# talmolab/VNL-Brax-Imitation

Measured on AMD Instinct MI355X. Metric: env-steps/sec (whole node), rodent imitation, num_envs=4096/GPU, higher is better.
Workload: dtype f32; 1 GPU; rodent imitation rollout, single groom clip, 4096 envs/GPU: intention-policy forward (HIP) -> RodentTracking.step (5 substeps, CG 6/6) -> auto-reset on -> Transition logging (unroll 20, the 20 steps replayed as one captured hipGraph); envs_per_gpu=4096, clips=1, parallelism=env-sharded x1, no data-path collective

## Files before the change

### __graft_entry__.py

```python
from __future__ import annotations

import os
import sys

ROOT = os.path.dirname(os.path.abspath(__file__))
if ROOT not in sys.path:
    sys.path.insert(0, ROOT)


def build() -> None:
    import vnl_brax_imitation_amd
    from vnl_brax_imitation_amd.csrc import build as hip_build

    from concurrent.futures import ThreadPoolExecutor

    with ThreadPoolExecutor(6) as pool:
        futs = {v: pool.submit(hip_build.build, variant=v) for v in ("product", "spill", "noblk", "nospec", "tail", "plain")}
        paths = {v: f.result() for v, f in futs.items()}
    path = paths["product"]
    assert all(os.path.exists(p_) for p_ in paths.values()), paths
    from oracle import oracle as _oracle

    _oracle.build()
    from vnl_brax_imitation_amd import _lib

    _lib.load_library(path)
    print(f"[build] {path} ok; oracle ok")


def smoke() -> None:
    import numpy as np
    import torch

    sys.path.insert(0, os.path.join(ROOT, "tests"))
    import helpers as H
    from vnl_brax_imitation_amd.envs.rodent import RodentTracking

    assert torch.cuda.is_available(), "smoke() needs a HIP device"
    B = 256
    env = RodentTracking(H.reference_clip(), num_envs=B, device="cuda:0", **H.env_kwargs())
# ... 43 lines not shown
```

### vnl-brax-imitation_amd/csrc/build.py

```python
from __future__ import annotations

import os
import subprocess
import sys

HERE = os.path.dirname(os.path.abspath(__file__))
SOURCES = ["vnl_lib.hip", "vnl_policy.hip", "vnl_ppo.hip", "vnl_domain.hip"]
DEPS = SOURCES + ["vnl_env_kernels.h", "vnl_body.h", "vnl_types.h", "vnl_philox.h", "vnl_policy_train.h", "../../include/vnl.h"]
OUT = os.path.join(HERE, "libvnl.so")

VARIANTS = {
    "product": ("libvnl.so", ["-DVNL_KERNEL_ATTR=__attribute__((amdgpu_waves_per_eu(2,2)))"]),
    "prof": ("libvnl_prof.so", ["-DVNL_PROFILE", "-DVNL_KERNEL_ATTR=__attribute__((amdgpu_waves_per_eu(2,2)))"]),
    "knobs": ("libvnl_knobs.so", ["-DVNL_STAGE_KNOBS", "-DVNL_KERNEL_ATTR=__attribute__((amdgpu_waves_per_eu(2,2)))"]),
    "spill": ("libvnl_spill.so", ["-DVNL_KERNEL_ATTR=__attribute__((amdgpu_waves_per_eu(4,4)))"]),
    "noblk": ("libvnl_noblk.so", ["-DVNL_NO_BLK", "-DVNL_KERNEL_ATTR=__attribute__((amdgpu_waves_per_eu(2,2)))"]),
    "tail": ("libvnl_tail.so", ["-DVNL_SOLVER_TAIL", "-DVNL_KERNEL_ATTR=__attribute__((amdgpu_waves_per_eu(2,2)))"]),
    "plain": ("libvnl_plain.so", ["-DVNL_SOLVER_PLAIN", "-DVNL_KERNEL_ATTR=__attribute__((amdgpu_waves_per_eu(2,2)))"]),
    "nospec": ("libvnl_nospec.so", ["-DVNL_NO_SPEC", "-DVNL_KERNEL_ATTR=__attribute__((amdgpu_waves_per_eu(2,2)))"]),
}
ENV_KERNELS = ("vnl_step_kernel", "vnl_reset_kernel", "vnl_reset_done_kernel")


def resource_usage(stderr_text: str) -> dict:
    out, name = {}, None
    for line in stderr_text.splitlines():
        if "Function Name:" in line:
            name = line.split("Function Name:")[1].split()[0]
            out[name] = {}
        elif name and "remark:" in line:
            body = line.split("remark:")[1].split("[-Rpass")[0].strip()
            key, _, val = body.rpartition(":")
            try:
                out[name][key.strip()] = int(val.strip())
            except ValueError:
                pass
    return out


def build(force: bool = False, verbose: bool = False, profile: bool = False, knobs: bool = False,
          variant: str | None = None) -> str:
# ... 78 lines not shown
```

### vnl-brax-imitation_amd/csrc/vnl_body.h

```cpp
#pragma once
#include <math.h>

#include "vnl_types.h"

#ifndef VNL_HD
#define VNL_HD __device__ __forceinline__
#endif
#include "vnl_philox.h"

#ifndef VNL_FORKJOIN_DEFINED
#define VNL_LANES 64
#define VNL_ROWS_PER_LANE 8
#define VNL_ROWS_SMALL 5
#define VNL_CHAIN_WIDTH 8
#define VNL_ROWSETS_1 1
#define VNL_ROWSETS_2 2
#define VNL_FOR(i, n) for (int i = (int)lane; i < (n); i += VNL_LANES)
#define VNL_SERIAL if (lane == 0)
#define VNL_SYNC() __builtin_amdgcn_fence(__ATOMIC_ACQ_REL, "wavefront")
#define VNL_SYNC_GLOBAL()                                     \
  do {                                                        \
    __builtin_amdgcn_fence(__ATOMIC_ACQ_REL, "wavefront");    \
    asm volatile("s_waitcnt vmcnt(0)" ::: "memory");          \
    __builtin_amdgcn_fence(__ATOMIC_ACQ_REL, "wavefront");    \
// ... 134 lines not shown
  return V3{m.a[0] * v.x + m.a[1] * v.y + m.a[2] * v.z, m.a[3] * v.x + m.a[4] * v.y + m.a[5] * v.z,
            m.a[6] * v.x + m.a[7] * v.y + m.a[8] * v.z};
}
struct S6 {
  V3 a, l;
};
VNL_HD S6 operator+(S6 p, S6 q) { return S6{p.a + q.a, p.l + q.l}; }
VNL_HD S6 operator*(S6 p, vreal s) { return S6{p.a * s, p.l * s}; }
VNL_HD vreal dot(S6 p, S6 q) { return dot(p.a, q.a) + dot(p.l, q.l); }
VNL_HD S6 mcross(S6 u, S6 v) { return S6{cross(u.a, v.a), cross(u.l, v.a) + cross(u.a, v.l)}; }
VNL_HD S6 mcross_force(S6 v, S6 f) { return S6{cross(v.a, f.a) + cross(v.l, f.l), cross(v.a, f.l)}; }

#if defined(__HIP_DEVICE_COMPILE__)
#define VNL_CAS __attribute__((address_space(4)))
#define VNL_TO_CAS(T, p) ((const VNL_CAS T*)(unsigned long long)(p))
#define VNL_LAUNDER(p) asm volatile("" : "+s"(p))
#else
#define VNL_CAS
#define VNL_TO_CAS(T, p) ((const T*)(p))
#define VNL_LAUNDER(p)
#endif
#define MI(f) (SP::fixed ? SP::D.f : m.f)
#define LO(f) (SP::fixed ? SP::L.f : L.f)
#if defined(__HIP_DEVICE_COMPILE__) && !defined(VNL_SOLVER_PLAIN)
#define VNL_SOLVE_REGS 1
#else
#define VNL_SOLVE_REGS 0
#endif
#define VNL_BLK_REGS 2
#define VNL_LIMROW_REGS 2
#define VNL_SR_BLK 1
#define VNL_SR_LIMROW 2
struct VnlSolveRegs {
  int on;
  unsigned blk[2][VNL_BLK_REGS];
  int limrow[VNL_LIMROW_REGS];
};
template <class SP>
struct EnvWaveT {
  const VNL_CAS DevModel& m;
  const VNL_CAS DevEnv& ev;
  const DevState& st;
  const VNL_CAS WsLayout& L;
  vreal* s;
  unsigned e, lane;
  const VNL_CAS KernelConsts* kc;
// ... 55 lines not shown

  VNL_HD V3 ld3(int o) const { return V3{s[o], s[o + 1], s[o + 2]}; }
  VNL_HD void st3(int o, V3 v) const { s[o] = v.x, s[o + 1] = v.y, s[o + 2] = v.z; }
  VNL_HD Q4 ld4(int o) const { return Q4{s[o], s[o + 1], s[o + 2], s[o + 3]}; }
  VNL_HD S6 ld6(int o) const { return S6{ld3(o), ld3(o + 3)}; }
  VNL_HD void st6(int o, S6 v) const { st3(o, v.a), st3(o + 3, v.l); }
  VNL_HD static V3 t3(const vreal* t, int i) { return V3{t[3 * i], t[3 * i + 1], t[3 * i + 2]}; }
  VNL_HD static Q4 t4(const vreal* t, int i) { return Q4{t[4 * i], t[4 * i + 1], t[4 * i + 2], t[4 * i + 3]}; }

  VNL_HD S6 inert_mul(int o, S6 v) const {
    vreal ixx = s[o], iyy = s[o + 1], izz = s[o + 2], ixy = s[o + 3], ixz = s[o + 4], iyz = s[o + 5];
    V3 mp = ld3(o + 6);
    vreal mass = s[o + 9];
    V3 ang = V3{ixx * v.a.x + ixy * v.a.y + ixz * v.a.z, ixy * v.a.x + iyy * v.a.y + iyz * v.a.z,
                ixz * v.a.x + iyz * v.a.y + izz * v.a.z} +
             cross(mp, v.l);
    V3 lin = v.l * mass - cross(mp, v.a);
    return S6{ang, lin};
  }

  VNL_HD vreal* gxpos() const { return st.xpos + (size_t)e * 3 * MI(nbody_out); }
  VNL_HD vreal* gxquat() const { return st.xquat + (size_t)e * 4 * MI(nbody_out); }
  VNL_HD vreal* gqfrc_act() const { return st.qfrc_actuator + (size_t)e * MI(nv); }
  VNL_HD vreal* fac2() const { return ev.fac2 + (size_t)e * (MI(nM) + MI(nv)); }
  enum { P_MU, P_INVW, P_GAIN, P_DAMP, P_ARM, P_MASS, P_IPOS, P_INERTIA6 };
  template <int F>
  VNL_HD vreal par(int i) const {
    if constexpr (SP::dom) {
      const VNL_CAS DevDomain& d = kc->dom;
      if constexpr (F == P_MU) return d.cg_mu[(size_t)e * MI(ncg) + i];
      else if constexpr (F == P_INVW) return d.cg_invweight[(size_t)e * MI(ncg) + i];
      else if constexpr (F == P_GAIN) return d.act_gain[(size_t)e * MI(nu) + i];
      else if constexpr (F == P_DAMP) return d.dof_damping[(size_t)e * MI(nv) + i];
      else return d.dof_armature[(size_t)e * MI(nv) + i];
    } else {
      if constexpr (F == P_MU) return m.cg_mu[i];
      else if constexpr (F == P_INVW) return m.cg_invweight[i];
      else if constexpr (F == P_GAIN) return m.act_gain[i];
      else if constexpr (F == P_DAMP) return m.dof_damping[i];
      else return m.dof_armature[i];
    }
  }
  template <int F>
  VNL_HD const vreal* par_row() const {
    if constexpr (SP::dom) {
      const VNL_CAS DevDomain& d = kc->dom;
      if constexpr (F == P_MASS) return d.body_mass + (size_t)e * MI(nbody);
// ... 590 lines not shown
#pragma unroll
          for (int u = 1; u < t; u++) acc -= nn[u] * x[u];
          nn[t] = acc;
        }
      }
      VNL_SYNC();
#pragma unroll
      for (int t = 1; t < MAXD; t++)
        if (t < qd(q) && t <= d) s[own + t] = nn[t];
      VNL_SYNC();
    }
  }

  template <int NSET>
  VNL_HD void factor_aba(vreal h) const {
    constexpr int LW = 16;
    const int sc = (LO(Mgrad) + 3) & ~3;
    const int VS = vstore();
    vreal* g2 = fac2();
    const int nsteps = MI(fac_steps);
    v2r U[NSET][6], diag[NSET];
    vreal S[NSET][6];
    int dep[NSET], ftime[NSET], myline[NSET], adrs[NSET];
    const unsigned char* mt[NSET];
    unsigned nxt[NSET];
#pragma unroll
    for (int q = 0; q < NSET; q++) {
      const int a = (int)lane + q * VNL_LANES;
      const bool ok = a < MI(nv);
      const int aa = ok ? a : 0;
      const S6 c = ld6(LO(cdof) + 6 * aa), f = inert_mul(LO(P) + 10 * m.dof_body[aa], c);
      S[q][0] = c.a.x, S[q][1] = c.a.y, S[q][2] = c.a.z, S[q][3] = c.l.x, S[q][4] = c.l.y, S[q][5] = c.l.z;
      U[q][0] = v2r{f.a.x, f.a.x}, U[q][1] = v2r{f.a.y, f.a.y}, U[q][2] = v2r{f.a.z, f.a.z};
      U[q][3] = v2r{f.l.x, f.l.x}, U[q][4] = v2r{f.l.y, f.l.y}, U[q][5] = v2r{f.l.z, f.l.z};
      const vreal arm = par<P_ARM>(aa);
      diag[q] = v2r{arm, arm + h * par<P_DAMP>(aa)};
      adrs[q] = madr(aa), dep[q] = eadr(aa) - adrs[q];
      myline[q] = m.dof_fslot[aa];
      ftime[q] = ok ? m.dof_ftime[aa] : -1;
      mt[q] = m.fac_match + (size_t)aa * nsteps;
      nxt[q] = (ok && nsteps > 0) ? mt[q][0] : 0u;
    }
    VNL_SYNC();
    VNL_PROF(7);
    for (int step = 0; step < nsteps; step++) {
      unsigned cur[NSET];
#pragma unroll
      for (int q = 0; q < NSET; q++) {
        cur[q] = nxt[q];
        nxt[q] = (ftime[q] >= 0 && step + 1 < nsteps) ? mt[q][step + 1] : 0u;
        if (ftime[q] == step) {
          const int a = (int)lane + q * VNL_LANES;
          v2r D = diag[q];
#pragma unroll
          for (int i = 0; i < 6; i++) D += v2r{S[q][i], S[q][i]} * U[q][i];
          const v2r iv = v2r{vnl_recip(D[0]), vnl_recip(D[1])};
          vreal* ln = s + sc + myline[q] * LW;
          st4a(ln, U[q][0][0], U[q][0][1], U[q][1][0], U[q][1][1]);
          st4a(ln + 4, U[q][2][0], U[q][2][1], U[q][3][0], U[q][3][1]);
          st4a(ln + 8, U[q][4][0], U[q][4][1], U[q][5][0], U[q][5][1]);
          st4a(ln + 12, iv[0], iv[1], (vreal)(adrs[q] + dep[q]), vreal(0.));
          vreal* vs = s + VS + 12 * a;
          const v2r v0 = U[q][0] * iv, v1 = U[q][1] * iv, v2 = U[q][2] * iv, v3_ = U[q][3] * iv, v4 = U[q][4] * iv, v5 = U[q][5] * iv;
          st4a(vs, v0[0], v0[1], v1[0], v1[1]);
          st4a(vs + 4, v2[0], v2[1], v3_[0], v3_[1]);
          st4a(vs + 8, v4[0], v4[1], v5[0], v5[1]);
          s[LO(dinv) + a] = iv[0];
          g2[MI(nM) + a] = iv[1];
        }
      }
      VNL_WAVE_FENCE();
      for (int pass = 0; pass < VNL_FAC_LINES; pass++) {
        bool more = false;
#pragma unroll
        for (int q = 0; q < NSET; q++) more = more || cur[q] != 0u;
        if (!vnl_wave_any(more)) break;
#pragma unroll
        for (int q = 0; q < NSET; q++) {
          if (cur[q] != 0u) {
            const int k = __builtin_ctz(cur[q]);
            cur[q] &= cur[q] - 1u;
            const vreal* ln = s + sc + k * LW;
            const R4 u0 = ld4a(ln), u1 = ld4a(ln + 4), u2 = ld4a(ln + 8), hd = ld4a(ln + 12);
            const v2r Uk[6] = {v2r{u0.x, u0.y}, v2r{u0.z, u0.w}, v2r{u1.x, u1.y}, v2r{u1.z, u1.w}, v2r{u2.x, u2.y}, v2r{u2.z, u2.w}};
            v2r pa = v2r{S[q][0], S[q][0]} * Uk[0], pb = v2r{S[q][1], S[q][1]} * Uk[1];
            pa += v2r{S[q][2], S[q][2]} * Uk[2], pb += v2r{S[q][3], S[q][3]} * Uk[3];
            pa += v2r{S[q][4], S[q][4]} * Uk[4], pb += v2r{S[q][5], S[q][5]} * Uk[5];
            const v2r Lk = (pa + pb) * v2r{hd.x, hd.y};
#pragma unroll
            for (int i = 0; i < 6; i++) U[q][i] -= Lk * Uk[i];
            s[LO(LD) + (int)hd.z - dep[q]] = Lk[0];
          }
        }
      }
      VNL_WAVE_FENCE();
    }
    VNL_SYNC();
    VNL_PROF(8);
    VNL_PROF(9);
  }

  VNL_HD int vstore() const { return vnl_vstore(LO(P)); }
  VNL_HD int cvel_at() const { return vnl_cvel_at(LO(P), LO(smooth), MI(nbody), MI(nv)); }

  template <int NSET, bool GUESTS>
  VNL_HD void invert_aba(vreal* g2) const {
    const int VS = vstore();
    const unsigned char* an = (const unsigned char*)(s + LO(tab_anc));
    auto load_v = [&](int r, v2r* C) {
      const vreal* vs = s + VS + 12 * r;
      const R4 a = ld4a(vs), b = ld4a(vs + 4), c = ld4a(vs + 8);
      C[0] = v2r{a.x, a.y}, C[1] = v2r{a.z, a.w}, C[2] = v2r{b.x, b.y}, C[3] = v2r{b.z, b.w}, C[4] = v2r{c.x, c.y}, C[5] = v2r{c.z, c.w};
    };
#pragma unroll
    for (int q = 0; q < NSET; q++) {
      const int a = (int)lane + q * VNL_LANES;
      int row = a < MI(nv) ? a : -1, next = -1;
      if (GUESTS && q == 0 && m.fac_guest) next = m.fac_guest[lane];
      int adr = madr(row >= 0 ? row : 0), d = row >= 0 ? eadr(row) - adr : 0, tt = 0;
// ... 302 lines not shown
    VNL_FOR(b, MI(nbody)) st6(ca + 6 * b, path_sum(QB, m.body_pathseg + 8 * b + 4));
    VNL_SYNC();
    VNL_PROF(3);
    VNL_FOR(b, MI(nbody)) {
      if (b == 0) {
        st6(ca, S6{v3(0, 0, 0), v3(0, 0, 0)});
        continue;
      }
      S6 vel = ld6(cv + 6 * b), acc = ld6(ca + 6 * b);
      acc.l = acc.l + v3(-m.gx, -m.gy, -m.gz);
      st6(ca + 6 * b, inert_mul(LO(P) + 10 * b, acc) + mcross_force(vel, inert_mul(LO(P) + 10 * b, vel)));
    }
    VNL_SYNC();
    tree_accumulate(ca, 6);
    VNL_FOR(d, MI(nv))
      s[LO(smooth) + d] = -par<P_DAMP>(d) * s[LO(qvel) + d] - dot(ld6(LO(cdof) + 6 * d), ld6(ca + 6 * m.dof_body[d]));
    VNL_SYNC();
    VNL_PROF(4);
    return cv;
  }

  VNL_HD void smooth_forces() const {
    VNL_FOR(j, MI(njnt)) {
      if (m.jnt_type[j] == VNL_JNT_HINGE) {
        vreal k = m.jnt_stiffness[j];
        if (k != vreal(0.)) s[LO(smooth) + m.jnt_dofadr[j]] -= k * (s[LO(qpos) + m.jnt_qposadr[j]] - m.jnt_springref[j]);
      }
    }
    const int frc = LO(tmp2), adof = LO(tmp);
    const bool listed = m.dof_act != nullptr;
    VNL_FOR(i, MI(nu)) {
      vreal ctrl = s[LO(ctrl) + i], a = ctrl;
      vreal tau = m.act_tau[i];
      if (tau >= vreal(0.)) {
        a = s[LO(act) + i];
        s[LO(actdot) + i] = (ctrl - a) / fmax(tau, VNL_MINVAL);
      }
      s[frc + i] = m.act_gear[i] * par<P_GAIN>(i) * a;
      if (!listed) s[adof + i] = vreal(m.act_dof[i]);
    }
    VNL_SYNC();
    vreal* gf = gqfrc_act();
    VNL_FOR(d, MI(nv)) {
      vreal fa = vreal(0.);
      if (listed) {
        for (unsigned pk = (unsigned)m.dof_act[d]; pk != 0u; pk >>= 8) fa += s[frc + (int)(pk & 0xffu) - 1];
      } else {
        const vreal me = vreal(d);
#pragma unroll 6
        for (int i = 0; i < MI(nu); i++) {
// ... 580 lines not shown
      if (newton) fresh().newton_solve(LO(tmp));
      else fresh().solve_inplace(LO(tmp));
      VNL_PROF(24);
      vreal d2 = vdot(LO(grad), LO(tmp));
      vreal beta = fmax(vreal(0.), (d2 - d1) / fmax(VNL_MINVAL, gp));
      if (newton) beta = vreal(0.);
      gp = d2;
      ss = vreal(0.);
      VNL_FOR(d, nv) {
        vreal mg = s[LO(tmp) + d];
        s[LO(Mgrad) + d] = mg;
        const vreal sn = -mg + beta * s[LO(search) + d];
        s[LO(search) + d] = sn;
        s[LO(mv) + d] = -s[LO(grad) + d] + beta * s[LO(mv) + d];
        ss += sn * sn;
      }
      ss = vnl_wave_sum(ss);
      VNL_SYNC();
      if (newton) fresh().newton_mass_mul(LO(search), LO(mv));
      VNL_PROF(25);
    }
  }

  VNL_HD void forward(const vreal* warm) const {
    VNL_FOR(d, MI(nv)) s[LO(tmp) + d] = warm[d];
    VNL_SYNC();
    VNL_FOR(d, MI(nv)) s[LO(qacc) + d] = s[LO(tmp) + d];
    VNL_SYNC();
#ifdef VNL_STAGE_KNOBS
    for (int rep = 0; rep < m.dbg_count; rep++) {
      if (m.dbg_stage == 1) {
        kinematics();
        body_inertias(false);
        mass_matrix(vreal(0.));
        factor();
        invert_factor();
      } else if (m.dbg_stage == 2) {
        kinematics();
      } else if (m.dbg_stage == 3) {
        kinematics();
        body_inertias(false);
        mass_matrix(vreal(0.));
      } else if (m.dbg_stage == 4) {
        kinematics();
        body_inertias(false);
        mass_matrix(vreal(0.));
        factor();
      } else if (m.dbg_stage == 5) {
        kinematics();
        body_inertias(true);
        (void)bias_forces();
// ... 75 lines not shown
        vreal c = constraint_force();
        if (c == vreal(-1.)) s[LO(tmp)] = c;
      } else if (m.dbg_stage == 11) {
        smooth_forces();
      } else if (m.dbg_stage == 12) {
        vreal c = vdot(LO(smooth), LO(qacc_smooth)) + vdot(LO(qacc), LO(smooth)) + vdot(LO(qacc), LO(qacc)) + vdot(LO(smooth), LO(smooth));
        if (c == vreal(-1.)) s[LO(tmp)] = c;
      } else if (m.dbg_stage == 13) {
        LsRows<VNL_ROWS_SMALL> rows;
        ls_load(rows, false);
        vreal a1[1] = {vreal(1e-4)};
        LsPoint p;
        ls_eval<1>(rows, a1, vreal(0.), vreal(0.), vreal(0.), &p);
        if (p.cost == vreal(-1.)) s[LO(tmp)] = p.cost;
      }
    }
#endif
    w.solve();
  }

  VNL_HD void euler() const {
    const int nv = MI(nv);
    VNL_PROF(26);
    VNL_FOR(d, nv) s[LO(tmp) + d] = MI(eulerdamp) ? s[LO(smooth) + d] + s[LO(qfrc_c) + d] : s[LO(qacc) + d];
    VNL_SYNC();
    if (MI(eulerdamp) && factor_pair_ok()) {
      const vreal* g2 = fac2();
      const int n2 = MI(nM) + MI(nv);
      VNL_SYNC_GLOBAL();
      VNL_FOR(k, n2) s[LO(P) + k] = g2[k];
      VNL_SYNC();
      fresh().with_solve_regs(false).solve_inplace(LO(tmp), LO(P), LO(P) + MI(nM));
      VNL_PROF(27);
    } else if (MI(eulerdamp)) {
      fresh().body_inertias(false);
      VNL_PROF(1);
      fresh().mass_matrix(m.dt);
      fresh().factor();
      fresh().invert_factor();
      fresh().with_solve_regs(false).solve_inplace(LO(tmp));
      VNL_PROF(27);
    }
    VNL_FOR(i, MI(nu)) {
      if (m.act_tau[i] >= vreal(0.)) s[LO(act) + i] += s[LO(actdot) + i] * m.dt;
    }
    VNL_FOR(d, nv) s[LO(qvel) + d] += s[LO(tmp) + d] * m.dt;
    VNL_SYNC();
    VNL_FOR(j, MI(njnt)) {
      int qa = m.jnt_qposadr[j], da = m.jnt_dofadr[j];
      if (m.jnt_type[j] == VNL_JNT_FREE) {
        for (int t = 0; t < 3; t++) s[LO(qpos) + qa + t] += m.dt * s[LO(qvel) + da + t];
        V3 w = ld3(LO(qvel) + da + 3);
        vreal nrm = sqrt(dot(w, w));
        V3 ax = nrm > vreal(0.) ? w * (vreal(1.) / nrm) : w;
        vreal ang = m.dt * nrm, sn = sin(vreal(0.5) * ang), cs = cos(vreal(0.5) * ang);
        Q4 r = qmul(ld4(LO(qpos) + qa + 3), Q4{cs, ax.x * sn, ax.y * sn, ax.z * sn});
        vreal n2 = sqrt(r.w * r.w + r.x * r.x + r.y * r.y + r.z * r.z);
        vreal inv = n2 > vreal(0.) ? vreal(1.) / n2 : vreal(1.);
        s[LO(qpos) + qa + 3] = r.w * inv, s[LO(qpos) + qa + 4] = r.x * inv, s[LO(qpos) + qa + 5] = r.y * inv,
                        s[LO(qpos) + qa + 6] = r.z * inv;
      } else {
        s[LO(qpos) + qa] += m.dt * s[LO(qvel) + da];
      }
    }
    VNL_SYNC();
// ... 130 lines not shown
    VNL_SYNC();
    fresh().kinematics();
    fresh().body_inertias(true);
    VNL_FOR(i, 3) st.com1[(size_t)e * 3 + i] = s[LO(com) + i];
    VNL_FOR(k, 4) st.qpos[(size_t)e * MI(nq) + 3 + k] = s[LO(qpos) + 3 + k];
  }

  template <bool KEEP_TERMINAL>
  VNL_HD void reset_core(const int* start_frame, const vreal* noise, int* trace_base) const {
    load_tables();
    int clip = st.clip_id[e], sf = start_frame[e];
    int f = clampi(sf, 0, ev.T - 1), nj = MI(nq) - 7;
    size_t fb = (size_t)clip * ev.T + f;
    const vreal* nz = noise + (size_t)e * MI(nq);
    VNL_FOR(k, 3) s[LO(qpos) + k] = vreal(ev.position[fb * 3 + k]) + nz[k];
    VNL_FOR(k, 4) s[LO(qpos) + 3 + k] = vreal(ev.quaternion[fb * 4 + k]) + nz[3 + k];
    VNL_FOR(k, nj) s[LO(qpos) + 7 + k] = vreal(ev.joints[fb * nj + k]) + nz[7 + k];
    VNL_FOR(k, 3) s[LO(qvel) + k] = ev.velocity[fb * 3 + k];
    VNL_FOR(k, 3) s[LO(qvel) + 3 + k] = ev.angular_velocity[fb * 3 + k];
    VNL_FOR(k, nj) s[LO(qvel) + 6 + k] = ev.joints_velocity[fb * nj + k];
    VNL_FOR(i, MI(nu)) s[LO(act) + i] = vreal(0.), s[LO(ctrl) + i] = vreal(0.);
    VNL_FOR(d, MI(nv)) s[LO(qacc) + d] = vreal(0.);
    VNL_SYNC();
    with_trace(trace_of(trace_base, 0)).forward(s + LO(qacc));
    VNL_SYNC_GLOBAL();
    store_state();
    write_traj(clip, sf);
    write_obs();
    vreal term = termination(clip, sf, s + LO(qpos), gxpos());
    VNL_SERIAL {
      if (!KEEP_TERMINAL) {
        st.reward[e] = vreal(0.), st.done[e] = vreal(0.);
        for (int k = 0; k < 7; k++) st.metrics[(size_t)e * 7 + k] = vreal(0.);
      }
      st.cur_frame[e] = sf, st.sub_clip_frame[e] = 0;
      st.term_err[e] = term;
    }
  }
  VNL_HD void reset(const int* start_frame, const vreal* noise, int* trace_base) const {
    reset_core<false>(start_frame, noise, trace_base);
  }

  VNL_HD void reset_fresh(const ResetDoneArgs& a, int* trace_base) const {
    const int nq = MI(nq), nblk = (nq + 3) >> 2;
    const int64_t step = *a.step_base + a.step_offset;
    const uint32_t c1 = a.env0 + (uint32_t)e, c2 = (uint32_t)step, c3 = ((uint32_t)(step >> 32) << 2) | 3u;
    vreal* nz = a.noise + (size_t)e * nq;
// ... 71 lines not shown
    prof_begin();
    int clip = st.clip_id[e], old_frame = st.cur_frame[e], old_sub = st.sub_clip_frame[e];
    load_tables();
    load_state();
    vreal rtrunk = termination(clip, old_frame, s + LO(qpos), gxpos());
    const vreal* ac = action + (size_t)e * MI(nu);
    VNL_FOR(i, MI(nu)) {
      vreal c = ac[i];
      if (m.act_limited[i]) c = c < m.act_lo[i] ? m.act_lo[i] : (c > m.act_hi[i] ? m.act_hi[i] : c);
      s[LO(ctrl) + i] = c;
    }
    VNL_SYNC();
    const vreal* gw = st.warm + (size_t)e * MI(nv);
    if (ev.flags & VNL_ENV_REWARD_OLD_STATE) {
      const RewardTerms r0 = reward_terms(clip, old_frame, s + LO(qpos), s + LO(qvel), st.com1 + (size_t)e * 3, gqfrc_act(), gxpos(), ac);
      VNL_SERIAL {
        vreal* mt = st.metrics + (size_t)e * 7;
        mt[0] = r0.rcom, mt[1] = r0.rvel, mt[2] = r0.rquat, mt[3] = r0.ract, mt[4] = r0.rapp, mt[5] = r0.healthy;
      }
      VNL_SYNC_GLOBAL();
    }
    VNL_PROF(29);
    for (int f = 0; f < ev.n_frames; f++) {
      fresh().with_trace(trace_of(trace_base, f)).forward(f == 0 ? gw : s + LO(qacc));
      if (dump_mid && f == ev.n_frames - 1) dump(dump_mid);
      fresh().euler();
    }
    int new_frame = old_frame + 1, new_sub = old_sub + 1;
    VNL_SYNC_GLOBAL();
    RewardTerms rw;
    if (!(ev.flags & VNL_ENV_REWARD_OLD_STATE)) {
      rw = reward_terms(clip, old_frame, s + LO(qpos), s + LO(qvel), s + LO(com), gqfrc_act(), gxpos(), ac);
    } else {
      const vreal* mt = st.metrics + (size_t)e * 7;
      rw = RewardTerms{mt[0], mt[1], mt[2], mt[3], mt[4], mt[5]};
      VNL_SYNC_GLOBAL();
    }
    const vreal done_trunk = rtrunk < ev.done_threshold ? vreal(1.) : vreal(0.);
    const vreal wcom = rw.rcom * ev.w_reward[0], wvel = rw.rvel * ev.w_reward[1], wtrunk = rtrunk * ev.w_reward[2];
    const vreal wquat = rw.rquat * ev.w_reward[3], wact = rw.ract * ev.w_reward[4], wapp = rw.rapp * ev.w_reward[5];
    const vreal total = wcom + wvel + wtrunk + wquat + wact + wapp;
    const bool raw = ev.flags & VNL_ENV_METRICS_UNSCALED;
    const vreal rcom = raw ? rw.rcom : wcom, rvel = raw ? rw.rvel : wvel, rquat = raw ? rw.rquat : wquat;
    const vreal ract = raw ? rw.ract : wact, rapp = raw ? rw.rapp : wapp;
    if (!raw) rtrunk = wtrunk;
    vreal done = fmax(vreal(1.) - rw.healthy, done_trunk);
    done = fmax(new_sub < ev.sub_clip_length ? vreal(0.) : vreal(1.), done);
// ... 23 lines not shown
```

### vnl-brax-imitation_amd/csrc/vnl_lib.hip

```cpp
#include <hip/hip_runtime.h>
#include <stdint.h>
#include <stdio.h>
#include <stdlib.h>
#include <string.h>

#include <algorithm>
#include <cmath>
#include <cstddef>
#include <map>
#include <string>
#include <vector>

#include "../../include/vnl.h"
#include "vnl_body.h"

static thread_local char g_err[512] = "";
static int fail(int code, const char* fmt, const char* a = "", const char* b = "") {
  snprintf(g_err, sizeof(g_err), fmt, a, b);
  return code;
}
#define HIPCHK(call)                                                              \
  do {                                                                            \
    hipError_t e_ = (call);                                                       \
    if (e_ != hipSuccess) return fail(VNL_ERR_HIP, "%s: %s", #call, hipGetErrorString(e_)); \
// ... 581 lines not shown
    {
      int deep1 = 0;
      for (int j = 64; j < nv; j++) deep1 = depth[j] > deep1 ? depth[j] : deep1;
      d.fac_route = choose_routes(d, deep1);
    }
    {
      d.fac_guest = nullptr;
      if (nv > 64 && nv <= 128) {
        std::vector<int> guest(64, -1), order;
        for (int j = 64; j < nv; j++) order.push_back(j);
        std::sort(order.begin(), order.end(), [&](int x, int y) { return depth[x] > depth[y]; });
        bool ok = true;
        for (int j : order) {
          int host = -1;
          for (int l = 0; l < 64 && host < 0; l++)
            if (guest[l] < 0 && depth[l] <= 12) host = l;
          if (host < 0 || depth[j] > 24) ok = false;
          else guest[host] = j;
        }
        if (ok) UPI(fac_guest, guest)
      }
    }
    {
      const int nst = d.fac_steps;
      std::vector<unsigned char> match((size_t)nv * (nst > 0 ? nst : 1), 0);
      for (int j = 0; j < nv; j++)
        for (int a = par[j]; a >= 0; a = par[a]) match[(size_t)a * nst + ftime[j]] |= (unsigned char)(1u << fslot[j]);
      const unsigned char* dp = nullptr;
      if ((rc = upload<unsigned char, unsigned char>(env, match, &dp)) != VNL_OK) return rc;
      d.fac_match = dp;
    }
    {
      d.blk_tab = nullptr, d.blk_cfg = 0;
      auto pack = [&](bool colform, std::vector<unsigned>& out, int& trips, int& steps) -> bool {
        struct Item { int r, nblk; };
        std::vector<Item> items;
        int total = 0, longest = 1;
        for (int r = 0; r < nv; r++) {
          const int len = colform ? ndesc[r] : depth[r], nb_ = len > 0 ? (len + VNL_BLK_W - 1) / VNL_BLK_W : 1;
          if (nb_ > 16) return false;
          items.push_back({r, nb_}), total += nb_, longest = nb_ > longest ? nb_ : longest;
        }
        std::stable_sort(items.begin(), items.end(), [](const Item& a, const Item& b) { return a.nblk > b.nblk; });
        steps = longest > 8 ? 4 : (longest > 4 ? 3 : (longest > 2 ? 2 : (longest > 1 ? 1 : 0)));
        for (trips = (total + 63) / 64; trips <= 8; trips++) {
          std::vector<int> fill(trips * 4, 0);
          std::vector<unsigned> tab((size_t)trips * 64, 0u);
          bool ok = true;
// ... 201 lines not shown
  }
  size_t CT = (size_t)e.C * e.T, nj = d.nq - 7;
#define UP(call)              \
  if ((rc = (call)) != VNL_OK) { \
    vnl_env_destroy(env);     \
    return rc;                \
  }
  UP(upload_raw<int>(env, es->body_idxs, e.nb, &e.body_idxs))
  UP(upload_raw<int>(env, es->end_eff_idx, e.nee, &e.end_eff_idx))
  UP(upload_raw<int>(env, es->app_body, e.napp, &e.app_body))
  UP(upload_raw<int>(env, es->app_ref_col, e.napp, &e.app_ref_col))
  UP(upload_raw<int>(env, es->joint_cols, e.njc, &e.joint_cols))
  UP(upload_raw<float>(env, es->position, CT * 3, &e.position))
  UP(upload_raw<float>(env, es->quaternion, CT * 4, &e.quaternion))
  UP(upload_raw<float>(env, es->joints, CT * nj, &e.joints))
  UP(upload_raw<float>(env, es->body_positions, CT * e.nb * 3, &e.body_positions))
  UP(upload_raw<float>(env, es->velocity, CT * 3, &e.velocity))
  UP(upload_raw<float>(env, es->angular_velocity, CT * 3, &e.angular_velocity))
  UP(upload_raw<float>(env, es->joints_velocity, CT * nj, &e.joints_velocity))
  if (es->center_of_mass) UP(upload_raw<float>(env, es->center_of_mass, CT * 3, &e.center_of_mass))
#undef UP
  {
    void* p = nullptr;
    HIPCHK(hipMalloc(&p, (size_t)num_envs * (d.nM + d.nv) * sizeof(vreal)));
    env->allocs.push_back(p);
    e.fac2 = (vreal*)p;
  }
  {
    void* p = nullptr;
    HIPCHK(hipMalloc(&p, (size_t)num_envs * (2 * sizeof(int) + d.nq * sizeof(vreal))));
    env->allocs.push_back(p);
    env->rd_noise = (vreal*)p;
    env->rd_start = (int*)(env->rd_noise + (size_t)num_envs * d.nq), env->rd_clip = env->rd_start + num_envs;
  }
  layout(env);
  env->spec = (same_dims(dims_of(env->dm), VnlSpecRodent::D) && same_layout(env->L, VnlSpecRodent::L)) ? 1 : 0;
#ifdef VNL_NO_SPEC
  env->spec = 0;
#endif
  env->lds_bytes = (size_t)env->L.total * sizeof(vreal);
#ifdef VNL_STAGE_KNOBS
  if (const char* padk = getenv("VNL_DBG_LDS_BYTES")) {
    size_t want = (size_t)atol(padk);
    if (want > env->lds_bytes) env->lds_bytes = want;
  }
#endif
  if (6 * d.nbody > 512) {
    vnl_env_destroy(env);
// ... 40 lines not shown
  o->factor_route = d.fac_route;
  return VNL_OK;
}

extern "C" int vnl_env_scratch(const vnl_env* env, const char* name, float** dev_ptr, int32_t* count) {
  if (!env || !name || !dev_ptr || !count) return fail(VNL_ERR_ARG, "vnl_env_scratch: null argument");
  if (strncmp(name, "dom_", 4) == 0) {
    if (!env->has_dom) return fail(VNL_ERR_ARG, "vnl_env_scratch: %s: the env has no domain (vnl_env_set_domain / vnl_env_set_body_domain)", name);
    const DevModel& d = env->dm;
    const size_t B = (size_t)env->B;
    const size_t n4 = B * (2 * d.ncg + d.nu + 2 * d.nv), nd = (size_t)d.nbody;
    const struct { const char* k; size_t off; int n; } tabs[] = {
        {"dom_mu", 0, d.ncg}, {"dom_invw", B * d.ncg, d.ncg}, {"dom_gain", 2 * B * d.ncg, d.nu},
        {"dom_damp", B * (2 * d.ncg + d.nu), d.nv}, {"dom_arm", B * (2 * d.ncg + d.nu + d.nv), d.nv},
        {"dom_mass", n4, d.nbody}, {"dom_ipos", n4 + B * nd, 3 * d.nbody}, {"dom_inertia6", n4 + 4 * B * nd, 6 * d.nbody},
        {"dom_tminv", n4 + 10 * B * nd, 1}};
    for (const auto& t : tabs)
      if (strcmp(name, t.k) == 0) {
        *dev_ptr = (float*)(env->dom + t.off);
        *count = t.n;
        return VNL_OK;
      }
    return fail(VNL_ERR_ARG, "unknown scratch section %s", name);
  }
  if (!env->dump) return fail(VNL_ERR_ARG, "scratch dump is off: call vnl_env_debug(env, 1) before reset/step");
  if (strcmp(name, "solver_trace") == 0) {
    *dev_ptr = (float*)env->trace;
    *count = (env->de.n_frames > 0 ? env->de.n_frames : 1) * VNL_TRACE_INTS;
    return VNL_OK;
  }
  auto it = env->sections.find(name);
  if (it == env->sections.end()) return fail(VNL_ERR_ARG, "unknown scratch section %s", name);
  *dev_ptr = (float*)(env->dump + it->second.first);
  *count = it->second.second;
  return VNL_OK;
}

extern "C" int vnl_env_debug(vnl_env* env, int32_t enable, int32_t* row_stride) {
  if (!env) return fail(VNL_ERR_ARG, "vnl_env_debug: null argument");
  if (enable < 0 || enable > 2) return fail(VNL_ERR_ARG, "vnl_env_debug: mode must be 0, 1 or 2");
  if (enable && !env->dump) {
    void* p = nullptr;
    HIPCHK(hipMalloc(&p, (size_t)env->L.total * env->B * sizeof(vreal)));
    env->allocs.push_back(p);
    env->dump = (vreal*)p;
    const size_t nt = (size_t)env->B * (env->de.n_frames > 0 ? env->de.n_frames : 1) * VNL_TRACE_INTS * sizeof(int);
// ... 680 lines not shown
```

### vnl-brax-imitation_amd/csrc/vnl_types.h

```cpp
#pragma once
#include <stdint.h>

#ifndef VNL_REAL
#define VNL_REAL float
#endif
typedef VNL_REAL vreal;

#define VNL_JNT_FREE 0
#define VNL_JNT_HINGE 3
#define VNL_GEOM_SPHERE 2
#define VNL_GEOM_CAPSULE 3
#define VNL_GEOM_ELLIPSOID 4

#define VNL_TRACE_ITERS 8
#define VNL_TRACE_REC 64
#define VNL_TRACE_ROWS (8 + VNL_TRACE_REC * VNL_TRACE_ITERS)
#define VNL_TRACE_INTS (VNL_TRACE_ROWS + 16)

#define VNL_LIVE_MAX 128
#define VNL_BLK_W 13
#define VNL_FAC_LINES 6

#define VNL_ROUTE_LDS 1
#define VNL_ROUTE_ROWS16 2
// ... 136 lines not shown
  L.tab_anc = sec(vnl_words(d.nM)), L.tab_madr = sec(vnl_words(6 * (long)d.nv));
  L.tab_body = sec(vnl_words(3 * (long)d.nbody + 2 * (long)d.ncon));
  L.tab_jump = sec(vnl_words((long)(d.jump_rounds > 0 ? d.jump_rounds : 1) * d.nbody));
  L.tab_lvl = sec(vnl_words((long)d.nv + d.max_depth + 2));
  L.act_list = sec(vnl_words(4 * (long)((d.ncon + 3) / 4) + 8 + 2 * VNL_LIVE_MAX));
  L.tab_con = sec(vnl_words(2 * (long)d.ncon)), L.tab_path = sec(vnl_words(2 * (long)d.path_runs * d.ncon));
  L.tab_lim = sec(vnl_words(d.nlimit)), L.con_mu = sec(d.ncg);
  L.newt_M = L.newt_H = 0;
  if (d.solver_newton) L.newt_M = sec(d.nM), L.newt_H = sec(d.nM + d.nv);
  if (VNL_NPROF_SLOTS) {
    o = (o + 1) & ~1;
    L.prof = sec(VNL_NPROF_SLOTS);
  }
  L.total = (o + 3) & ~3;
  return L;
}

constexpr int vnl_vstore(int P) { return (P + 3) & ~3; }
constexpr int vnl_cvel_at(int P, int smooth, int nbody, int nv) {
  const int a = P + 16 * nbody, b = vnl_vstore(P) + 12 * nv;
  return (b > a && b + 6 * nbody <= smooth) ? b : a;
}

struct VnlSpecGeneric {
  static constexpr bool fixed = false;
  static constexpr bool dom = false;
  static constexpr VnlDims D{};
  static constexpr WsLayout L{};
};
struct VnlSpecRodent {
  static constexpr bool fixed = true;
  static constexpr bool dom = false;
  static constexpr VnlDims D{74, 73, 30, 53, 68, 32, 59, 67, 303, 1119, 6, 6, 1, 1, 35, 5, 36,
                             VNL_ROUTE_ROWS36X2 | (VNL_ROUTE_ROWS36X2 << VNL_ROUTE_QM_INVERSE) | (2 << VNL_ROUTE_PAIR), 0,
                             2 | (2 << 4) | (2 << 8) | (3 << 12), 2, 66};
  static constexpr WsLayout L = vnl_make_layout(D);
};
template <class BASE>
struct VnlSpecDom : BASE {
  static constexpr bool dom = true;
};

struct DevDomain {
  const vreal *cg_mu, *cg_invweight;
  const vreal *act_gain;
  const vreal *dof_damping, *dof_armature;
// ... 12 lines not shown
```

Before: 2.548 million env-steps/s.

## Reshape factorization and warmstart global memory access for wider loads

The per-DOF factorization match table is padded to a multiple of four bytes and preloaded into registers as 32-bit words, which are shifted per step instead of issuing a byte load every step. The inverse diagonal writes to fac2 are deferred into registers and stored once after the loop. Euler's damped solve now copies the padded fac2 buffer into shared scratch with vectorized 4-wide global loads before solving in place. Forward skips the redundant warmstart round-trip when qacc is already resident, and joint parameters are pinned to registers in smooth_forces. These changes add register pressure and padding, and a plain build variant keeps the old path for comparison.

```diff
diff --git a/__graft_entry__.py b/__graft_entry__.py
--- a/__graft_entry__.py
+++ b/__graft_entry__.py
@@ -14,8 +14,9 @@
 
     from concurrent.futures import ThreadPoolExecutor
 
-    with ThreadPoolExecutor(6) as pool:
-        futs = {v: pool.submit(hip_build.build, variant=v) for v in ("product", "spill", "noblk", "nospec", "tail", "plain")}
+    with ThreadPoolExecutor(7) as pool:
+        futs = {v: pool.submit(hip_build.build, variant=v)
+                for v in ("product", "spill", "noblk", "nospec", "tail", "plain", "vmemplain")}
         paths = {v: f.result() for v, f in futs.items()}
     path = paths["product"]
     assert all(os.path.exists(p_) for p_ in paths.values()), paths
diff --git a/vnl-brax-imitation_amd/csrc/build.py b/vnl-brax-imitation_amd/csrc/build.py
--- a/vnl-brax-imitation_amd/csrc/build.py
+++ b/vnl-brax-imitation_amd/csrc/build.py
@@ -17,6 +17,7 @@
     "noblk": ("libvnl_noblk.so", ["-DVNL_NO_BLK", "-DVNL_KERNEL_ATTR=__attribute__((amdgpu_waves_per_eu(2,2)))"]),
     "tail": ("libvnl_tail.so", ["-DVNL_SOLVER_TAIL", "-DVNL_KERNEL_ATTR=__attribute__((amdgpu_waves_per_eu(2,2)))"]),
     "plain": ("libvnl_plain.so", ["-DVNL_SOLVER_PLAIN", "-DVNL_KERNEL_ATTR=__attribute__((amdgpu_waves_per_eu(2,2)))"]),
+    "vmemplain": ("libvnl_vmemplain.so", ["-DVNL_VMEM_PLAIN", "-DVNL_KERNEL_ATTR=__attribute__((amdgpu_waves_per_eu(2,2)))"]),
     "nospec": ("libvnl_nospec.so", ["-DVNL_NO_SPEC", "-DVNL_KERNEL_ATTR=__attribute__((amdgpu_waves_per_eu(2,2)))"]),
 }
 ENV_KERNELS = ("vnl_step_kernel", "vnl_reset_kernel", "vnl_reset_done_kernel")
diff --git a/vnl-brax-imitation_amd/csrc/vnl_body.h b/vnl-brax-imitation_amd/csrc/vnl_body.h
--- a/vnl-brax-imitation_amd/csrc/vnl_body.h
+++ b/vnl-brax-imitation_amd/csrc/vnl_body.h
@@ -180,6 +180,16 @@
 #endif
 #define MI(f) (SP::fixed ? SP::D.f : m.f)
 #define LO(f) (SP::fixed ? SP::L.f : L.f)
+#if defined(__HIP_DEVICE_COMPILE__)
+#define VNL_GLOBAL_PTR(T, p) ((const __attribute__((address_space(1))) T*)(p))
+#else
+#define VNL_GLOBAL_PTR(T, p) ((const T*)(p))
+#endif
+#if defined(__HIP_DEVICE_COMPILE__) && !defined(VNL_VMEM_PLAIN)
+#define VNL_PIN(x) asm volatile("" : "+v"(x))
+#else
+#define VNL_PIN(x) (void)(x)
+#endif
 #if defined(__HIP_DEVICE_COMPILE__) && !defined(VNL_SOLVER_PLAIN)
 #define VNL_SOLVE_REGS 1
 #else
@@ -281,7 +291,7 @@
   VNL_HD vreal* gxpos() const { return st.xpos + (size_t)e * 3 * MI(nbody_out); }
   VNL_HD vreal* gxquat() const { return st.xquat + (size_t)e * 4 * MI(nbody_out); }
   VNL_HD vreal* gqfrc_act() const { return st.qfrc_actuator + (size_t)e * MI(nv); }
-  VNL_HD vreal* fac2() const { return ev.fac2 + (size_t)e * (MI(nM) + MI(nv)); }
+  VNL_HD vreal* fac2() const { return ev.fac2 + (size_t)e * vnl_fac2_stride(MI(nM), MI(nv)); }
   enum { P_MU, P_INVW, P_GAIN, P_DAMP, P_ARM, P_MASS, P_IPOS, P_INERTIA6 };
   template <int F>
   VNL_HD vreal par(int i) const {
@@ -918,8 +928,30 @@
     v2r U[NSET][6], diag[NSET];
     vreal S[NSET][6];
     int dep[NSET], ftime[NSET], myline[NSET], adrs[NSET];
+#ifdef VNL_VMEM_PLAIN
     const unsigned char* mt[NSET];
     unsigned nxt[NSET];
+#else
+    constexpr int NW = SP::fixed ? vnl_imax(vnl_fac_stride(SP::D.fac_steps) / 4, 1) : 4;
+    const int nwords = vnl_fac_stride(nsteps) / 4;
+    const auto* mw = VNL_GLOBAL_PTR(unsigned, m.fac_match);
+    unsigned woff[NSET], win[NSET][NW], wcur[NSET];
+    auto pick_word = [&](int q, int i) {
+      unsigned r = win[q][0];
+#pragma unroll
+      for (int k = 1; k < NW; k++) {
+        unsigned w = win[q][k];
+        VNL_PIN(w);
+        r = i == k ? w : r;
+      }
+      return r;
+    };
+    auto load_window = [&](int q, bool ok, int w0) {
+#pragma unroll
+      for (int i = 0; i < NW; i++) win[q][i] = (ok && w0 + i < nwords) ? mw[woff[q] + (unsigned)(w0 + i)] : 0u;
+    };
+    vreal inv2[NSET];
+#endif
 #pragma unroll
     for (int q = 0; q < NSET; q++) {
       const int a = (int)lane + q * VNL_LANES;
@@ -934,8 +966,15 @@
       adrs[q] = madr(aa), dep[q] = eadr(aa) - adrs[q];
       myline[q] = m.dof_fslot[aa];
       ftime[q] = ok ? m.dof_ftime[aa] : -1;
-      mt[q] = m.fac_match + (size_t)aa * nsteps;
+#ifdef VNL_VMEM_PLAIN
+      mt[q] = m.fac_match + (size_t)aa * vnl_fac_stride(nsteps);
       nxt[q] = (ok && nsteps > 0) ? mt[q][0] : 0u;
+#else
+      woff[q] = (unsigned)(aa * nwords);
+      load_window(q, ok, 0);
+      wcur[q] = win[q][0];
+      inv2[q] = vreal(0.);
+#endif
     }
     VNL_SYNC();
     VNL_PROF(7);
@@ -943,8 +982,12 @@
       unsigned cur[NSET];
 #pragma unroll
       for (int q = 0; q < NSET; q++) {
+#ifdef VNL_VMEM_PLAIN
         cur[q] = nxt[q];
         nxt[q] = (ftime[q] >= 0 && step + 1 < nsteps) ? mt[q][step + 1] : 0u;
+#else
+        cur[q] = wcur[q] & 0xffu, wcur[q] >>= 8;
+#endif
         if (ftime[q] == step) {
           const int a = (int)lane + q * VNL_LANES;
           v2r D = diag[q];
@@ -962,7 +1005,11 @@
           st4a(vs + 4, v2[0], v2[1], v3_[0], v3_[1]);
           st4a(vs + 8, v4[0], v4[1], v5[0], v5[1]);
           s[LO(dinv) + a] = iv[0];
+#ifdef VNL_VMEM_PLAIN
           g2[MI(nM) + a] = iv[1];
+#else
+          inv2[q] = iv[1];
+#endif
         }
       }
       VNL_WAVE_FENCE();
@@ -990,7 +1037,22 @@
         }
       }
       VNL_WAVE_FENCE();
-    }
+#ifndef VNL_VMEM_PLAIN
+      if ((step & 3) == 3) {
+        const int wi = (step >> 2) + 1;
+#pragma unroll
+        for (int q = 0; q < NSET; q++) {
+          if (!SP::fixed && wi % NW == 0) load_window(q, ftime[q] >= 0, wi);
+          wcur[q] = pick_word(q, wi % NW);
+        }
+      }
+#endif
+    }
+#ifndef VNL_VMEM_PLAIN
+#pragma unroll
+    for (int q = 0; q < NSET; q++)
+      if (ftime[q] >= 0) g2[MI(nM) + (int)lane + q * VNL_LANES] = inv2[q];
+#endif
     VNL_SYNC();
     VNL_PROF(8);
     VNL_PROF(9);
@@ -1339,10 +1401,17 @@
 
   VNL_HD void smooth_forces() const {
     VNL_FOR(j, MI(njnt)) {
+#ifdef VNL_VMEM_PLAIN
       if (m.jnt_type[j] == VNL_JNT_HINGE) {
         vreal k = m.jnt_stiffness[j];
         if (k != vreal(0.)) s[LO(smooth) + m.jnt_dofadr[j]] -= k * (s[LO(qpos) + m.jnt_qposadr[j]] - m.jnt_springref[j]);
       }
+#else
+      int type = m.jnt_type[j], da = m.jnt_dofadr[j], qa = m.jnt_qposadr[j];
+      vreal k = m.jnt_stiffness[j], ref = m.jnt_springref[j];
+      VNL_PIN(type); VNL_PIN(da); VNL_PIN(qa); VNL_PIN(k); VNL_PIN(ref);
+      if (type == VNL_JNT_HINGE && k != vreal(0.)) s[LO(smooth) + da] -= k * (s[LO(qpos) + qa] - ref);
+#endif
     }
     const int frc = LO(tmp2), adof = LO(tmp);
     const bool listed = m.dof_act != nullptr;
@@ -1969,11 +2038,20 @@
     }
   }
 
-  VNL_HD void forward(const vreal* warm) const {
+  VNL_HD void forward(const vreal* gwarm) const {
+#ifdef VNL_VMEM_PLAIN
+    const vreal* warm = gwarm ? gwarm : s + LO(qacc);
     VNL_FOR(d, MI(nv)) s[LO(tmp) + d] = warm[d];
     VNL_SYNC();
     VNL_FOR(d, MI(nv)) s[LO(qacc) + d] = s[LO(tmp) + d];
     VNL_SYNC();
+#else
+    if (gwarm) {
+      const auto* gw = VNL_GLOBAL_PTR(vreal, gwarm);
+      VNL_FOR(d, MI(nv)) s[LO(qacc) + d] = gw[d];
+      VNL_SYNC();
+    }
+#endif
 #ifdef VNL_STAGE_KNOBS
     for (int rep = 0; rep < m.dbg_count; rep++) {
       if (m.dbg_stage == 1) {
@@ -2095,6 +2173,42 @@
   VNL_HD void euler() const {
     const int nv = MI(nv);
     VNL_PROF(26);
+#ifndef VNL_VMEM_PLAIN
+    if (MI(eulerdamp) && factor_pair_ok()) {
+      constexpr int NB = SP::fixed ? (vnl_fac2_stride(SP::D.nM, SP::D.nv) / 4 + VNL_LANES - 1) / VNL_LANES : 4;
+      const auto* g2 = VNL_GLOBAL_PTR(vreal, fac2());
+      const int n2 = MI(nM) + MI(nv), n2p = vnl_fac2_stride(MI(nM), MI(nv));
+      VNL_SYNC_GLOBAL();
+      bool rhs = false;
+      for (int k0 = 4 * (int)lane; !rhs || k0 < n2p; k0 += 4 * VNL_LANES * NB) {
+        R4 x[NB];
+#pragma unroll
+        for (int t = 0; t < NB; t++) {
+          const int k = k0 + 4 * VNL_LANES * t;
+          if (k < n2p) x[t] = ld4a(g2 + k);
+        }
+        if (!rhs) {
+          VNL_FOR(d, nv) s[LO(tmp) + d] = s[LO(smooth) + d] + s[LO(qfrc_c) + d];
+          rhs = true;
+        }
+#pragma unroll
+        for (int t = 0; t < NB; t++) {
+          const int k = k0 + 4 * VNL_LANES * t;
+          if (k + 3 < n2) {
+            s[LO(P) + k] = x[t].x, s[LO(P) + k + 1] = x[t].y, s[LO(P) + k + 2] = x[t].z, s[LO(P) + k + 3] = x[t].w;
+          } else if (k < n2) {
+            s[LO(P) + k] = x[t].x;
+            if (k + 1 < n2) s[LO(P) + k + 1] = x[t].y;
+            if (k + 2 < n2) s[LO(P) + k + 2] = x[t].z;
+          }
+        }
+      }
+      VNL_SYNC();
+      fresh().with_solve_regs(false).solve_inplace(LO(tmp), LO(P), LO(P) + MI(nM));
+      VNL_PROF(27);
+    } else
+#endif
+    {
     VNL_FOR(d, nv) s[LO(tmp) + d] = MI(eulerdamp) ? s[LO(smooth) + d] + s[LO(qfrc_c) + d] : s[LO(qacc) + d];
     VNL_SYNC();
     if (MI(eulerdamp) && factor_pair_ok()) {
@@ -2114,6 +2228,7 @@
       fresh().with_solve_regs(false).solve_inplace(LO(tmp));
       VNL_PROF(27);
     }
+    }
     VNL_FOR(i, MI(nu)) {
       if (m.act_tau[i] >= vreal(0.)) s[LO(act) + i] += s[LO(actdot) + i] * m.dt;
     }
@@ -2290,7 +2405,7 @@
     VNL_FOR(i, MI(nu)) s[LO(act) + i] = vreal(0.), s[LO(ctrl) + i] = vreal(0.);
     VNL_FOR(d, MI(nv)) s[LO(qacc) + d] = vreal(0.);
     VNL_SYNC();
-    with_trace(trace_of(trace_base, 0)).forward(s + LO(qacc));
+    with_trace(trace_of(trace_base, 0)).forward(nullptr);
     VNL_SYNC_GLOBAL();
     store_state();
     write_traj(clip, sf);
@@ -2408,7 +2523,7 @@
     }
     VNL_PROF(29);
     for (int f = 0; f < ev.n_frames; f++) {
-      fresh().with_trace(trace_of(trace_base, f)).forward(f == 0 ? gw : s + LO(qacc));
+      fresh().with_trace(trace_of(trace_base, f)).forward(f == 0 ? gw : nullptr);
       if (dump_mid && f == ev.n_frames - 1) dump(dump_mid);
       fresh().euler();
     }
diff --git a/vnl-brax-imitation_amd/csrc/vnl_lib.hip b/vnl-brax-imitation_amd/csrc/vnl_lib.hip
--- a/vnl-brax-imitation_amd/csrc/vnl_lib.hip
+++ b/vnl-brax-imitation_amd/csrc/vnl_lib.hip
@@ -627,8 +627,8 @@
       }
     }
     {
-      const int nst = d.fac_steps;
-      std::vector<unsigned char> match((size_t)nv * (nst > 0 ? nst : 1), 0);
+      const int nst = vnl_fac_stride(d.fac_steps);
+      std::vector<unsigned char> match((size_t)nv * (nst > 0 ? nst : 4), 0);
       for (int j = 0; j < nv; j++)
         for (int a = par[j]; a >= 0; a = par[a]) match[(size_t)a * nst + ftime[j]] |= (unsigned char)(1u << fslot[j]);
       const unsigned char* dp = nullptr;
@@ -876,8 +876,10 @@
 #undef UP
   {
     void* p = nullptr;
-    HIPCHK(hipMalloc(&p, (size_t)num_envs * (d.nM + d.nv) * sizeof(vreal)));
+    const size_t n2 = (size_t)num_envs * vnl_fac2_stride(d.nM, d.nv) * sizeof(vreal);
+    HIPCHK(hipMalloc(&p, n2));
     env->allocs.push_back(p);
+    HIPCHK(hipMemset(p, 0, n2));
     e.fac2 = (vreal*)p;
   }
   {
@@ -964,6 +966,11 @@
         return VNL_OK;
       }
     return fail(VNL_ERR_ARG, "unknown scratch section %s", name);
+  }
+  if (strcmp(name, "fac_match") == 0) {
+    *dev_ptr = (float*)env->dm.fac_match;
+    *count = vnl_fac_stride(env->dm.fac_steps) / 4;
+    return VNL_OK;
   }
   if (!env->dump) return fail(VNL_ERR_ARG, "scratch dump is off: call vnl_env_debug(env, 1) before reset/step");
   if (strcmp(name, "solver_trace") == 0) {
diff --git a/vnl-brax-imitation_amd/csrc/vnl_types.h b/vnl-brax-imitation_amd/csrc/vnl_types.h
--- a/vnl-brax-imitation_amd/csrc/vnl_types.h
+++ b/vnl-brax-imitation_amd/csrc/vnl_types.h
@@ -182,6 +182,9 @@
   return (b > a && b + 6 * nbody <= smooth) ? b : a;
 }
 
+constexpr int vnl_fac_stride(int fac_steps) { return (fac_steps + 3) & ~3; }
+constexpr int vnl_fac2_stride(int nM, int nv) { return (nM + nv + 3) & ~3; }
+
 struct VnlSpecGeneric {
   static constexpr bool fixed = false;
   static constexpr bool dom = false;
```

Result: faster. 2.582 million env-steps/s, median of 6 (+1.3%).
